# TUMFTM/GraphBasedLocalTrajectoryPlanner

Measured on AMD Instinct MI355X. Metric: planning ticks/s (all action primitives), Monteblanco lattice, higher is better.
Workload: dtype f64; 1 GPU; C2: Monteblanco lattice (128 layers / 2691 nodes / 14264 edges), 4 action primitives, 8 dynamic opponents (16 obstacle positions), sample zone; 32768 independent scenarios per GPU per step, tick pipeline (paths + velocity); batch_per_gpu=32768, batch_total=32768, parallelism=scenario-sharded x1 (no collective; results stay on the ranks)

## Files before the change

graphbasedlocaltrajectoryplanner_amd/csrc/ltpl_hip.hip:

```cpp
#include <hip/hip_runtime.h>
#include <algorithm>
#include <atomic>
#include <cmath>
#include <cstddef>
#include <cstdint>
#include <cstdio>
#include <cstdlib>
#include <cstring>
#include <exception>
#include <memory>
#include <string>
#include <type_traits>
#include <vector>

#include "../../include/ltpl_hip.h"
#include "planner_host.hpp"
#include "fleet_api.hpp"
#include "capsule.hpp"
#include "layer_grid.hpp"
#include "assembly_records.hpp"

#define WG_THREADS 256
#define PIPELINE_MIN_SCEN 64
#define NUM_WAVES 4
// ... 4 lines not shown
#define F_DEF 1
#define F_LEFT 2
#define F_RIGHT 3
#define D_PI 3.14159265358979323846

#define LTPL_SW_PAD 512
struct DevLat {
    int L, V, E, S, G;
    int mode;
    int closed;
    double min_plan_horizon, veh_width, sampled_resolution, lat_offset, vel_decrease_lat, veh_length;
    const int* layer_off; const int* rl_idx;
    const double* s_rl; const double* ref_x; const double* ref_y; const double* vel_rl;
    const double* node_x; const double* node_y; const double* vgoal;
    const int* in_ptr; const int* edge_src; const double* edge_cost; const double* edge_len; const int* samp_ptr;
    const double* sx; const double* sy; const double* spsi; const double* slen;
    const double* ssc;
    const double* glob_rl;
    const double* grx; const double* gry;
    const int* rng_end;
    const int* layer_ebase;
    const unsigned char* edge_src8;
    const unsigned char* edge_dst8;
    const unsigned char* edge_rank8;
    const int* layer_degmax;
    const double* sw_cost;
    const unsigned* sw_meta;
    const int* sw2csc;
    const int* csc2sw;
    const double* b1x; const double* b1y; const double* b2x; const double* b2y; const double* ctx; const double* cty;
    const float4* edge_cap;
    float cull_slack;
    const int4* lgrid; double lg_x0, lg_y0, lg_inv; int lg_nx, lg_ny;
    const int4* node_rec;
    const double* edge_rec;
};

struct DevPathsIn {
    int n_scen, n_w_last;
    const double* w_last;
    const int* start_layer; const int* start_node; const int* flags; const int* last_action; const int* const_closest;
    const double* psi_s;
    const int* veh_off; const int* pos_off; const double* veh_radius; const double* pos_x; const double* pos_y;
    const int* zone_off; const int* zone_gid;
    const int* n_last; const int* last_layer; const int* last_node;
    const int* order;
};

struct DoneSignal { unsigned* host_flag; unsigned* dev_count; unsigned seq; };

__device__ __forceinline__ void signal_done(const DoneSignal& d)
{
    if (!d.host_flag) return;
    __threadfence_system();
    __syncthreads();
    if (threadIdx.x == 0) {
        const unsigned prev = atomicAdd(d.dev_count, 1u);
        if (prev == gridDim.x - 1) {
            *d.dev_count = 0u;
            __hip_atomic_store(d.host_flag, d.seq, __ATOMIC_RELEASE, __HIP_MEMORY_SCOPE_SYSTEM);
        }
    }
}

#ifndef LTPL_VEL_F32_OPERANDS
typedef double ke_scalar;
// ... 555 lines not shown
    const double t = ((px - ax) * (bx - ax) + (py - ay) * (by - ay)) / ((bx - ax) * (bx - ax) + (by - ay) * (by - ay));
    const double fx = ax + t * (bx - ax), fy = ay + t * (by - ay);
    const double ds = sqrt((ax - fx) * (ax - fx) + (ay - fy) * (ay - fy));
    const double s = (ord > 0 ? s_arr[(size_t)i1 * s_stride] : s_arr[(size_t)nb * s_stride]) + ds;
    if (idx0) *idx0 = (ord >= 0) ? i1 : nb;
    return s;
}

__device__ __forceinline__ int globrl_index_dev(const DevLat& lat, double px, double py, int lane)
{
    const int G = lat.G - 1;
    double bd = INFINITY; int nb = 0x7fffffff;
    for (int i0 = 0; i0 < G; i0 += 256) {
        double xs[4], ys[4]; int id[4];
#pragma unroll
        for (int u = 0; u < 4; ++u) { const int i = i0 + u * 64 + lane; id[u] = i < G ? i : G - 1; xs[u] = at(lat.grx, id[u]); ys[u] = at(lat.gry, id[u]); }
#pragma unroll
        for (int u = 0; u < 4; ++u) {
            const double dx = xs[u] - px, dy = ys[u] - py, d2 = dx * dx + dy * dy;
            if (d2 < bd) { bd = d2; nb = id[u]; }
        }
    }
    wave_min2(bd, nb);
    int i1 = nb - 1; if (i1 < 0) i1 += G;
    int i2 = nb + 1; if (i2 > G - 1) i2 = 0;
    const int ord = angle_order_dev(at(lat.grx, nb), at(lat.gry, nb), px, py, at(lat.grx, i1), at(lat.gry, i1), at(lat.grx, i2), at(lat.gry, i2));
    return ord >= 0 ? i1 : nb;
}

__device__ __forceinline__ int lane_globrl_index(const DevLat& lat, double ox, double oy)
{
    const int G = lat.G - 1;
    double bd = INFINITY; int nb = 0;
#pragma unroll 8
    for (int i = 0; i < G; ++i) {
        const double dx = lat.grx[i] - ox, dy = lat.gry[i] - oy, d2 = dx * dx + dy * dy;
        if (d2 < bd) { bd = d2; nb = i; }
    }
    int i1 = nb - 1; if (i1 < 0) i1 += G;
    int i2 = nb + 1; if (i2 > G - 1) i2 = 0;
    const int ord = angle_order_dev(at(lat.grx, nb), at(lat.gry, nb), ox, oy, at(lat.grx, i1), at(lat.gry, i1), at(lat.grx, i2), at(lat.gry, i2));
    return ord >= 0 ? i1 : nb;
}

struct FollowIn { double v_start, v_ego, v_obj, safety_d, obj_dist, obj_x, obj_y; };

template <int EM, bool AXM1, bool GGARR>
__device__ __forceinline__ void follow_profile(const DevLat& lat, int n, int n_el, const VelScratch& vs, double cax, double cay,
                               const DevVelParams& p, const FollowIn& fi, int lane, int* too_close, int* vel_bound,
                               bool ext_sync = false, bool skip_free = false)
{
    int vb = 1;
    const double control_d = p.c_p * fi.safety_d + p.len_veh;
    const double safety_d = fi.safety_d + p.len_veh;
    const int tc = (fi.obj_dist - safety_d) < 0.0;
    const double v_max = p.v_max;

    dbg_stamp(vs.dbg, 4);
    brake_profile<EM, GGARR>(n, vs.wb, vs, cax, cay, fi.v_start, p, lane);
    dbg_stamp(vs.dbg, 5);
    wave_cumsum_seq(vs.el, vs.s, n_el, lane);
    int idb = wave_find_first(n, lane, [&](int i) { return !(vs.wb[i] > 0.01); });
    if (idb > n_el) idb = n_el;
    double ego_stop = 0.0;
    if (idb > 0) ego_stop = (idb < n_el) ? vs.s[idb] : vs.s[n_el - 1] + vs.el[n_el - 1];

    const int G = lat.G - 1;
    const double* grl = lat.glob_rl;
    dbg_stamp(vs.dbg, 6);
    const int idx_s_opp = globrl_index_dev(lat, fi.obj_x, fi.obj_y, lane);
// ... 491 lines not shown
    for (int pass = 0; pass < 4; ++pass) {
        const int half = pass & 1;
        if ((lane >> 5) == half) {
#pragma unroll
            for (int c = 0; c < NCH; c += 2) store2(&E.tbuf[(lane & 31) * PITCH + c], pass < 2 ? vv[c] : aa[c], pass < 2 ? vv[c + 1] : aa[c + 1]);
        }
        wave_sync_lds();
#pragma unroll
        for (int k = 0; k < 4; ++k) {
            const int jl = k * 8 + q, jj = half * 32 + jl, c = 2 * piece;
            const int cn = E.s_cnt[jj];
            if (c >= cn || c >= NCH) continue;
            const dbl2 v = *reinterpret_cast<const dbl2*>(&E.tbuf[jl * PITCH + c]);
            double* o = reinterpret_cast<double*>(E.s_o[jj]) + (pass < 2 ? 0 : E.ax_delta) + (E.s_rhi[jj] - c);
            if (c + 1 < cn) store2_u(o - 1, v.y, v.x); else o[0] = v.x;
        }
        wave_sync_lds();
    }
}

struct NoCap { static constexpr bool active = false; __device__ __forceinline__ double at(int) const { return INFINITY; } };
struct FollowCap {
    static constexpr bool active = true;
    const double* P2; const double* P3; int nd, stop_idx;
    __device__ __forceinline__ double at(int r) const
    {
        const bool from_b = nd < 0 || r < nd - 1;
        const double* src = from_b ? P2 : P3;
        const double v = src[(size_t)r * 64];
        return (!from_b && r > stop_idx) ? 0.0 : v;
    }
};

template <int EM, bool AXM1, bool EMIT = false, class CAP = NoCap>
__device__ __forceinline__ void lane_fb_profile(const LaneProf& L, double* D, int off, int n, double cax, double cay,
                                                const DevVelParams& p, const double* axm_tab, double v_max, double v_start,
                                                bool has_v_end, double v_end, long long* dbg = nullptr, int drow = -1, LaneEmit* em = nullptr, int lane = 0,
                                                const CAP& cap = CAP())
{
    if (v_start < 0.0) v_start = 0.0;
    if (has_v_end && v_end < 0.0) v_end = 0.0;
    const double vmax2 = v_max * v_max, icay = 1.0 / cay, axm1 = axm_tab[1], dm = p.drag_m, axa = fabs(cax);
    const double vend2 = has_v_end ? v_end * v_end : INFINITY;
    const ke_t* KEb = L.KE;
#define KE_AT(r) KEb[kep_row(off + (r))]
    double* Dp = D + (size_t)off * 64;
    const ke_t rec0 = KE_AT(0);
    double kabs_i = (double)rec0.x, e_i = (double)rec0.y;
    double wi = fmin(cay * ke_rcp(rec0), vmax2);
    if (wi > v_start * v_start) wi = v_start * v_start;
    Dp[0] = wi;
    if constexpr (!EMIT) { if (n < 2) return; }
    do {
    if constexpr (EMIT) { if (n < 2) break; }
    if constexpr (EM == 1 && AXM1) {
        constexpr int CA = CAP::active ? LCHC : LCHA;
        const double axg = axa * icay;
        double orig_p = wi, g_p = kabs_i * axg, e_p = e_i;
        bool active = false, prev_acc = false;
        ke_t kr[CA], kn[CA];
        const int nst = n - 1;
#pragma unroll
        for (int c = 0; c < CA; ++c) { const int r = 1 + c < n ? 1 + c : n - 1; kr[c] = KE_AT(r); }
        auto step = [&](const ke_t& rec, int i, bool valid) {
            const double w0n = fmin(cay * ke_rcp(rec), vmax2);
            const bool acc = w0n > orig_p;
            const bool act = active || (acc && !prev_acc);
            const double te = e_p + e_p;
            const double u = fmin(fmax(fma(-g_p, wi, axa), 0.0), axm1);
            const double wn = fmax(fma(te, u, fma(-(te * dm), wi, wi)), 0.0);
            const double wnext = (act && wn < w0n) ? wn : w0n;
            if (valid) {
                Dp[(size_t)(i + 1) * 64] = wnext;
                active = act && !(wn > vmax2); prev_acc = acc;
                wi = wnext; orig_p = w0n; g_p = (double)rec.x * axg; e_p = (double)rec.y;
            }
        };
        int base = 0;
        for (; base + CA <= nst; base += CA) {
#pragma unroll
            for (int c = 0; c < CA; ++c) {
                const int r = base + CA + 1 + c < n ? base + CA + 1 + c : n - 1;
                kn[c] = KE_AT(r);
            }
#pragma unroll
            for (int c = 0; c < CA; ++c) step(kr[c], base + c, true);
// ... 189 lines not shown
                    const double C0 = te * dm, C1 = C0 - te * (axa * kq_n), D1 = te * axa;
                    wn = fmax(fmax(fma(A1, wi, B1), A0 * wi), 0.0);
                    const double t0 = fma(C0, wn, wi), t1 = fma(C1, wn, wi + D1);
                    wn = fmin(fmax(fmax(t1, t0), 0.0), wn);
                } else {
                    const double a = ax_poss_w<EM, AXM1, VMODE_DECEL_BACKW>(wi, kq_i, cax, p, axm_tab, axm1);
                    wn = fmax(wi + 2.0 * a * e_b, 0.0);
                    const double a2 = ax_poss_w<EM, AXM1, VMODE_DECEL_BACKW>(wn, kq_n, cax, p, axm_tab, axm1);
                    wn = fmin(fmax(wi + 2.0 * a2 * e_b, 0.0), wn);
                }
                const bool take = act && wn < wold;
                const double wnext = take ? wn : wold;
                if (valid && take) Dp[(size_t)(n - 2 - i) * 64] = wn;
                const bool act_out = act && !(wn > vmax2);
                active = valid ? act_out : active; prev_acc = valid ? acc : prev_acc;
                orig_i = valid ? wold : orig_i; wi = valid ? wnext : wi; kabs_i = valid ? k_c : kabs_i;
            }
#pragma unroll
            for (int c = 0; c < LCHB; ++c) { kr[c] = kn[c]; wr[c] = wq[c]; }
        }
    }
}

#undef KE_AT

#define VF_BOUND_FOLLOW 1
#define VF_TOO_CLOSE    2
#define VF_HAS_GENERIC  4
#define VF_BOUND_GENERIC 8
#define VF_COMPOSE 16
#define VF_DONE 32

struct LaneFollowOut { int vel_bound, too_close, two_seg, n_decel, stop_idx; };
template <int EM, bool AXM1>
__device__ __forceinline__ LaneFollowOut lane_follow_controlled(const DevLat& lat, const LaneProf& L, double* P2, double* P3, int n, double cax, double cay,
                                                                const DevVelParams& p, const double* axm_tab, double v_start, double v_ego, double v_obj,
                                                                double obj_dist, double safety_d_in, int idx_s_opp, long long* dbg, int drow)
{
    const double icay = 1.0 / cay;
    int vel_bound = 1;
    const double control_d = p.c_p * safety_d_in + p.len_veh, safety_d = safety_d_in + p.len_veh;
    const int too_close = (obj_dist - safety_d) < 0.0 ? 1 : 0;
    const double v_max = p.v_max;
    double v_control;
    if (p.ctrl == 0) v_control = (v_obj - p.k_p * (control_d - obj_dist) + p.k_d * (v_obj - v_ego));
    else {
        double a = (control_d - obj_dist) * D_PI / 2 * 1 / p.tan_w;
        const double lo = -D_PI / 2 + 1e-5, hi = D_PI / 2 - 1e-5;
        a = a < lo ? lo : (a > hi ? hi : a);
        v_control = (v_obj - tan(a) * p.k_p + p.k_d * (v_obj - v_ego));
    }
    if (v_control < 0.0) v_control = 0.0;
    if (v_control > v_max) v_control = v_max;
    const double wctl = v_control * v_control;

    const int G = lat.G - 1;
    const double* grl = lat.glob_rl;
    const double vel0 = grl[(size_t)idx_s_opp * 5 + 4];
    double wopp = fmin(v_obj, vel0); wopp *= wopp;
    double opp_stop = 0.0;
    for (int base = 0; base < G && wopp > 0.01; base += LCH) {
        double kr[LCH], lr[LCH];
#pragma unroll
        for (int c = 0; c < LCH; ++c) {
            int j = base + c + idx_s_opp; j = j % G;
            kr[c] = fabs(grl[(size_t)j * 5 + 3]); lr[c] = grl[(size_t)(j + 1) * 5] - grl[(size_t)j * 5];
        }
#pragma unroll
        for (int c = 0; c < LCH; ++c) {
            const int k = base + c;
            if (k < G && wopp > 0.01) {
                opp_stop += lr[c];
                if (k + 1 >= G) wopp = 0.0;
                else {
                    const double a = ax_poss_w<EM, true, VMODE_DECEL_FORW>(wopp, kr[c] * (1.0 / 14.0), 14.0, p, axm_tab, 0.0);
                    const double r = wopp + 2.0 * a * lr[c];
                    wopp = r < 0.0 ? 0.0 : r;
                }
            }
        }
    }
    vl_stamp(dbg, drow, 1);
    const double s_stop = obj_dist - safety_d + opp_stop;
    double ego_stop = 0.0, s_run = 0.0, s_last = 0.0; int first_le = -1, stop_idx = 0;
    {
        double w = v_start * v_start; bool braking = true, counting = true, searching = true;
        double kr[LCH], er[LCH], kn[LCH], en[LCH];
        auto load_rows = [&](int base, double (&k)[LCH], double (&e)[LCH]) {
#pragma unroll
            for (int c = 0; c < LCH; ++c) {
                const int r = base + c < n ? base + c : n - 1;
                const ke_t ke = L.KE[kep_row(r)]; k[c] = (double)ke.x; e[c] = (double)ke.y;
            }
        };
        load_rows(0, kr, er);
        for (int base = 0; base < n; base += LCH) {
            if (base + LCH < n) load_rows(base + LCH, kn, en);
#pragma unroll
            for (int c = 0; c < LCH; ++c) {
                const int i = base + c;
                if (i < n) {
                    const double wv = braking ? w : 0.0;
                    P2[(size_t)i * 64] = wv;
                    if (first_le < 0 && wv <= wctl) first_le = i;
                    if (counting) { if (wv > 0.01) ego_stop += er[c]; else counting = false; }
                    if (searching) { if (i < n - 1 && s_run < s_stop) stop_idx = i + 1; else searching = false; }
                    if (i == n - 1) s_last = s_run;
                    s_run += er[c];
                    if (braking && i + 1 < n) {
                        const double kq = kr[c] * icay, e = er[c];
                        double r;
                        if constexpr (EM == 1) {
                            const double te = 2.0 * e, axa = fabs(cax);
                            const double A0 = 1.0 - te * p.drag_m, A1 = A0 + te * (axa * kq);
                            r = fmin(fma(A1, w, -te * axa), A0 * w);
                        } else {
                            r = w + 2.0 * ax_poss_w<EM, true, VMODE_DECEL_FORW>(w, kq, cax, p, axm_tab, 0.0) * e;
                        }
// ... 17 lines not shown
                int j = idx + c + idx_s_opp; j = j % G;
                dl[c] = grl[(size_t)(j + 1) * 5] - grl[(size_t)j * 5];
            }
#pragma unroll
            for (int c = 0; c < LCH; ++c)
                if (run) { if (summed < s_ends && idx < G) { summed += dl[c]; ++idx; } else run = false; }
            if (run && !(summed < s_ends && idx < G)) run = false;
        }
        int j = (idx % G) + idx_s_opp; if (j >= G) j -= G;
        v_end = grl[(size_t)j * 5 + 4];
    }
    vl_stamp(dbg, drow, 3);
    int idx_c = 0, n_decel = 0; const bool two_seg = ego_stop < s_stop;
    if (two_seg) {
        double vcs = v_start;
        if (v_start > v_control && stop_idx >= 2) {
            idx_c = first_le < 0 ? 0 : first_le;
            if (idx_c > stop_idx) idx_c = stop_idx;
            if (idx_c == 0) idx_c = stop_idx;
            n_decel = idx_c + 1 < n ? idx_c + 1 : n;
            vcs = sqrt(P2[(size_t)(n_decel - 1) * 64]);
        } else if (!(stop_idx >= 2)) vel_bound = 0;
        const int m = (stop_idx + 1 < n ? stop_idx + 1 : n) - idx_c;
        if (stop_idx - idx_c > 0) {
            lane_fb_profile<EM, AXM1>(L, P3, idx_c, m, cax, cay, p, axm_tab, v_control, vcs, true, v_end);
            if (fabs(sqrt(P3[(size_t)idx_c * 64]) - vcs) > 1.0) vel_bound = 0;
        } else if (stop_idx - idx_c == 0) P3[(size_t)idx_c * 64] = vcs * vcs;
        const double first_v = (n_decel - 1 > 0) ? sqrt(P2[0]) : sqrt(P3[0]);
        if (fabs(first_v - v_start) > 1.0) vel_bound = 0;
    }
    vl_stamp(dbg, drow, 4);
    LaneFollowOut o; o.vel_bound = vel_bound; o.too_close = too_close; o.two_seg = two_seg ? 1 : 0; o.n_decel = n_decel; o.stop_idx = stop_idx;
    return o;
}

template <int EM, bool AXM1>
__device__ __forceinline__ int lane_generic_profile(const DevLat& lat, const DevPathsOut& out, const LaneProf& L, double* D, int slot, int n,
                                    int reduced, double cax, double cay, const DevVelParams& p, const double* axm_tab,
                                    double vel_plan, double v_max_offset)
{
    const int goal = out.goal_layer[slot];
    const int end_node = out.nodes[(size_t)slot * out.cap_nodes + out.n_nodes[slot] - 1];
    int dn = end_node - lat.rl_idx[goal]; if (dn < 0) dn = -dn;
    const double raceline_offset = (double)dn * lat.lat_offset;
    double v_end; int v_idx;
    if (reduced) {
        v_end = 0.0;
        double spl_len = 0.0;
        for (int i = 0; i < n - 1; ++i) spl_len += (double)L.KE[kep_row(i)].y;
        int first = -1; double c = 0.0;
        for (int i = 0; i < n - 1; ++i) { c += (double)L.KE[kep_row(i)].y; if (first < 0 && !(c < (spl_len - 5.0))) first = i; }
        v_idx = (first < 0 ? 0 : first) + 1;
        if (v_idx == 1 && n > 1) v_idx = n;
    } else {
        v_end = lat.vel_rl[goal];
        const double red = v_end * lat.vel_decrease_lat * raceline_offset;
        v_end -= (red < v_end ? red : v_end);
        v_idx = n;
    }
    if (v_idx > 1) lane_fb_profile<EM, AXM1>(L, D, 0, v_idx, cax, cay, p, axm_tab, p.v_max, vel_plan, true, v_end);
    else D[0] = 0.0;
    for (int i = (v_idx > 1 ? v_idx : 1); i < n; ++i) D[(size_t)i * 64] = 0.0;
    return fabs(sqrt(D[0]) - vel_plan) < v_max_offset ? 1 : 0;
}

template <int EM, bool AXM1>
// ... 85 lines not shown
        LaneProf L; L.KE = vp.KE + kep_base(j, vp.plane_rows);
        double* o_vx = vout.vx + (size_t)slot * out.cap_pts;
        le_o[lane] = have ? (unsigned long long)o_vx : 0ull;
        LaneEmit E; E.tbuf = le_tbuf; E.s_cnt = le_cnt; E.s_rhi = le_rhi; E.s_o = le_o; E.ax_delta = (long long)(vout.ax - vout.vx); E.w0 = 0.0;
        wave_sync_lds();
        const int bound = lane_generic_profile_emit<EM, AXM1>(lat, out, L, vp.P0 + tile_base(j, vp.cap_pts), have, slot, n, have ? out.reduced[slot] : 0,
                                                              cax, cay, p, axm_tab, have ? vin.vel_plan[slot / LTPL_MAX_ACTIONS] : 0.0, vin.v_max_offset, E, lane, o_vx);
        if (have) {
            vout.vel_bound[slot] = bound; vout.too_close[slot] = 0;
            vp.flags[j] = VF_BOUND_FOLLOW | (bound ? VF_BOUND_GENERIC : 0);
        }
        vl_stamp(dbg, drow, 6);
        return;
    }
    if (b >= nbG && (emit & 2)) {
        const int j = (b - nbG) * 64 + lane;
        const bool have = j < cntF;
        const int tile = fbase + j;
        const int2 js = have ? out.job_slot[tile] : make_int2(0, 0);
        const int slot = js.x, n = have ? js.y : 0;
        {
            const int nmax = wave_max_i32(n);
            if (lane == 0) atomicMax(&out.job_cnt[2], nmax);
        }
        const int s = slot / LTPL_MAX_ACTIONS;
        LaneProf L; L.KE = vp.KE + kep_base(tile, vp.plane_rows);
        double* P2 = vp.P2 + tile_base(j, vp.cap_pts);
        double* P3 = vp.P3 + tile_base(j, vp.cap_pts);
        const double vel_plan = have ? vin.vel_plan[s] : 0.0;
        const int reduced = have ? out.reduced[slot] : 0;
        FollowCap cap; cap.P2 = P2; cap.P3 = P3; cap.nd = -1; cap.stop_idx = 0;
        bool direct = false;
        int o_bound = 0, o_close = 0;
        if (have) {
            const LaneFollowOut fo = lane_follow_controlled<EM, AXM1>(lat, L, P2, P3, n, cax, cay, p, axm_tab, vel_plan, vin.vel_est[s], prep.v_obj[slot],
                                                                      prep.obj_dist[slot], vin.safety_d, prep.idx_s_opp[slot], dbg, drow);
            o_bound = fo.vel_bound; o_close = fo.too_close;
            if (!reduced) { direct = true; cap.nd = fo.two_seg ? fo.n_decel : -1; cap.stop_idx = fo.stop_idx; }
            else {
                double* P0 = vp.P0 + tile_base(tile, vp.cap_pts);
                int flags = VF_BOUND_FOLLOW | VF_HAS_GENERIC;
                if (fo.too_close) flags |= VF_TOO_CLOSE;
                if (!fo.vel_bound) flags &= ~VF_BOUND_FOLLOW;
                const bool two_seg = fo.two_seg != 0;
                for (int i = 0; i < n; ++i) {
                    const bool from_b = !two_seg || i < fo.n_decel - 1;
                    P0[(size_t)i * 64] = from_b ? P2[(size_t)i * 64] : ((i > fo.stop_idx) ? 0.0 : P3[(size_t)i * 64]);
                }
                if (lane_generic_profile<EM, AXM1>(lat, out, L, P3, slot, n, reduced, cax, cay, p, axm_tab, vel_plan, vin.v_max_offset))
                    flags |= VF_BOUND_GENERIC;
                vp.flags[tile] = flags;
            }
        }
        double* o_vx = vout.vx + (size_t)slot * out.cap_pts;
        le_o[lane] = direct ? (unsigned long long)o_vx : 0ull;
        LaneEmit E; E.tbuf = le_tbuf; E.s_cnt = le_cnt; E.s_rhi = le_rhi; E.s_o = le_o; E.ax_delta = (long long)(vout.ax - vout.vx); E.w0 = 0.0;
        wave_sync_lds();
        double* D = direct ? vp.P1 + tile_base(j, vp.cap_pts) : P2;
        lane_fb_profile<EM, AXM1, true, FollowCap>(L, D, 0, direct && n >= 2 ? n : 0, cax, cay, p, axm_tab, p.v_max, vel_plan, false, 0.0, nullptr, -1, &E, lane, cap);
        if (direct) {
            const int i = n - 1;
            const double w = fmin(cap.at(i), D[(size_t)i * 64]);
            o_vx[i] = sqrt(w); o_vx[i + E.ax_delta] = 0.0;
            vout.vel_bound[slot] = o_bound; vout.too_close[slot] = o_close;
            vp.flags[tile] = VF_DONE;
        }
        vl_stamp(dbg, drow, 6);
        return;
    }
    const bool fjob = b >= nbG;
    const int j = (fjob ? b - nbG : b) * 64 + lane;
    if (j >= (fjob ? cntF : cntG)) return;
    const int tile = fjob ? fbase + j : j;
    const int2 js = out.job_slot[tile];
    const int slot = js.x;
    {
        int nmax = js.y;
#pragma unroll
        for (int m = 32; m >= 1; m >>= 1) { const int o = __shfl_xor(nmax, m); nmax = o > nmax ? o : nmax; }
        if (lane == 0) atomicMax(&out.job_cnt[2], nmax);
    }
    const int s = slot / LTPL_MAX_ACTIONS;
    const int n = js.y;
    LaneProf L; L.KE = vp.KE + kep_base(tile, vp.plane_rows);
    double* P0 = vp.P0 + tile_base(tile, vp.cap_pts);
    double* P2 = vp.P2 + tile_base(fjob ? j : 0, vp.cap_pts);
    double* P3 = vp.P3 + tile_base(fjob ? j : 0, vp.cap_pts);
    const double vel_plan = vin.vel_plan[s];
    const int name = out.action_id[slot], reduced = out.reduced[slot];
    int flags = VF_BOUND_FOLLOW;

    if (name == LTPL_ACT_FOLLOW) {
// ... 690 lines not shown

    ltpl_handle* h = new ltpl_handle();
    h->device = device;
    h->rng_end_host = rng_end;
    struct Guard { ltpl_handle* h; ~Guard() { if (h) ltpl_destroy(h); } } guard{h};
    auto fail = [&](int code) { g_create_error = h->err; return code; };
    if (hipSetDevice(device) != hipSuccess) { h->err = "hipSetDevice failed"; return fail(LTPL_ERR_HIP); }
    if (hipStreamCreateWithFlags(&h->stream, hipStreamNonBlocking) != hipSuccess) { h->err = "hipStreamCreate failed"; return fail(LTPL_ERR_HIP); }

    DevLat& L = h->lat;
    L.L = d->num_layers; L.V = d->num_nodes; L.E = d->num_edges; L.S = d->num_samples; L.G = d->num_glob_rl;
    L.mode = d->plan_horizon_mode; L.closed = d->closed ? 1 : 0; L.min_plan_horizon = d->min_plan_horizon; L.veh_width = d->veh_width;
    L.sampled_resolution = d->sampled_resolution; L.lat_offset = d->lat_offset;
    L.vel_decrease_lat = d->vel_decrease_lat; L.veh_length = d->veh_length;
#define UP(field, src, n) if ((rc = upload(h, src, (size_t)(n), &L.field)) != LTPL_OK) return fail(rc)
    UP(layer_off, d->layer_node_off, L.L + 1); UP(rl_idx, d->raceline_index, L.L);
    UP(s_rl, d->s_raceline, L.L); UP(ref_x, d->refline_x, L.L); UP(ref_y, d->refline_y, L.L);
    UP(vel_rl, d->vel_raceline, L.L);
    UP(node_x, d->node_x, L.V); UP(node_y, d->node_y, L.V); UP(vgoal, d->vgoal_cost, L.V);
    UP(in_ptr, d->in_ptr, L.V + 1); UP(edge_src, d->edge_src, L.E);
    UP(edge_cost, d->edge_cost, L.E);
    UP(edge_len, d->edge_len, L.E); UP(samp_ptr, d->samp_ptr, L.E + 1);
    UP(sx, d->samp_x, L.S); UP(sy, d->samp_y, L.S); UP(spsi, d->samp_psi, L.S); UP(slen, d->samp_len, L.S);
    UP(glob_rl, d->glob_rl, (size_t)L.G * 5);
    {
        std::vector<double> sc(2 * (size_t)L.S + 2, 0.0);
        for (int k = 0; k < L.S; ++k) { sc[2 * (size_t)k] = sin(d->samp_psi[k]); sc[2 * (size_t)k + 1] = cos(d->samp_psi[k]); }
        UP(ssc, sc.data(), 2 * (size_t)L.S + 2);
    }
    {
        std::vector<double> gx((size_t)L.G), gy((size_t)L.G);
        for (int k = 0; k < L.G; ++k) { gx[(size_t)k] = d->glob_rl[(size_t)k * 5 + 1]; gy[(size_t)k] = d->glob_rl[(size_t)k * 5 + 2]; }
        UP(grx, gx.data(), L.G); UP(gry, gy.data(), L.G);
    }
    {
        std::vector<int> ebase((size_t)L.L + 1);
        for (int l = 0; l <= L.L; ++l) ebase[(size_t)l] = d->in_ptr[d->layer_node_off[l]];
        std::vector<unsigned char> src8((size_t)L.E + 16, (unsigned char)0xff);
        for (int e = 0; e < L.E; ++e) src8[(size_t)e] = (unsigned char)d->edge_src[e];
        std::vector<unsigned char> dst8((size_t)L.E);
        for (int l = 0; l < L.L; ++l)
            for (int v = d->layer_node_off[l]; v < d->layer_node_off[l + 1]; ++v)
                for (int e = d->in_ptr[v]; e < d->in_ptr[v + 1]; ++e) dst8[(size_t)e] = (unsigned char)(v - d->layer_node_off[l]);
        UP(rng_end, rng_end.data(), L.L); UP(layer_ebase, ebase.data(), L.L + 1); UP(edge_src8, src8.data(), L.E + 16);
        UP(edge_dst8, dst8.data(), L.E);
        std::vector<unsigned char> rank8((size_t)L.E);
        for (int v = 0; v < L.V; ++v)
            for (int e = d->in_ptr[v]; e < d->in_ptr[v + 1]; ++e) rank8[(size_t)e] = (unsigned char)(e - d->in_ptr[v]);
        UP(edge_rank8, rank8.data(), L.E);
        {
            std::vector<int32_t> nrec; std::vector<double> erec;
            ltplrec::build(L.V, L.E, d->in_ptr, d->edge_src, d->edge_len, d->samp_ptr, d->samp_x, d->samp_y, d->samp_psi, nrec, erec);
            const int4* nr = nullptr;
            if ((rc = upload(h, reinterpret_cast<const int4*>(nrec.data()), (size_t)L.V, &nr)) != LTPL_OK) return fail(rc);
            L.node_rec = nr;
            UP(edge_rec, erec.data(), (size_t)L.E * LTPL_EDGE_REC);
        }
        std::vector<int> ldeg((size_t)L.L, 0);
        for (int l = 0; l < L.L; ++l)
            for (int v = d->layer_node_off[l]; v < d->layer_node_off[l + 1]; ++v)
                ldeg[(size_t)l] = std::max(ldeg[(size_t)l], d->in_ptr[v + 1] - d->in_ptr[v]);
        UP(layer_degmax, ldeg.data(), L.L);
        h->sw2csc_host.resize((size_t)L.E);
        std::vector<int> csc2sw((size_t)L.E);
        for (int l = 0; l < L.L; ++l) {
            const int e0 = ebase[(size_t)l], e1 = ebase[(size_t)l + 1];
// ... 690 lines not shown
    if (polled) done = next_done_signal(h);
    hipLaunchKernelGGL(kern, dim3(n_jobs), dim3(64), lds, h->stream, h->lat, p,
                       reinterpret_cast<const DevVelJob*>(db + o_jobs), reinterpret_cast<const double*>(db + o_pool),
                       reinterpret_cast<double*>(dob + o_vx), reinterpret_cast<int*>(dob + o_flags), cap, h->lp4.dbg, done, 1);
    HIP_TRY(h, hipGetLastError());
    if (!zc) HIP_TRY(h, hipMemcpyAsync(h->h_out, h->d_out, aout.size, hipMemcpyDeviceToHost, h->stream));
    prof_enq.stop();
    LTPL_PROF(prof_sync, "vel_profile.sync");
    if (polled) { if ((rc = wait_done(h, done.seq))) return rc; }
    else HIP_TRY(h, hipStreamSynchronize(h->stream));
    prof_sync.stop();
    dbg_report(h, "k_vel_profile", n_jobs);
    LTPL_PROF(prof_sc, "vel_profile.scatter");
    const unsigned char* ho = static_cast<const unsigned char*>(h->h_out);
    const int* flags = reinterpret_cast<const int*>(ho + o_flags);
    const double* vx = reinterpret_cast<const double*>(ho + o_vx);
    for (int j = 0; j < n_jobs; ++j) {
        memcpy(results[j].vx, vx + dj[(size_t)j].off_out, sizeof(double) * (size_t)jobs[j].n);
        results[j].too_close = flags[2 * j]; results[j].vel_bound = flags[2 * j + 1];
    }
    return LTPL_OK;
} LTPL_ABI_CATCH(abi_err_of(h))

struct TickLayout {
    InLayout in; size_t axm, vel_plan, vel_est, pos_x, pos_y, veh_vel, in_total;
    OutLayout out; size_t vx, ax, vel_bound, too_close, out_total;
    int n_scen, cap_nodes, cap_pts;
    DevPathsIn di; DevPathsOut dout; DevVelParams p; DevTickVelIn dvin; DevTickVelOut dvout;
    int vel_off, vel_stride, vel_cap; size_t lds;
    int variant;
    bool pipeline; size_t prep_odist, prep_vobj, prep_ox, prep_oy, prep_idx; size_t planes_bytes;
    DevVelPrep dprep; int prep_off, prep_stride;
    VelPlanes vp{}; int n_slots_pad = 0, n_scen_pad = 0;
};

static int tick_prepare(ltpl_handle* h, const ltpl_paths_in* in, const ltpl_tick_vel_in* vin, int cap_nodes, int cap_pts,
                        TickLayout* t)
{
    int rc = validate_and_layout(h, in, &t->in);
    if (rc) return rc;
    if (!vin || !vin->params) { h->err = "velocity inputs missing"; return LTPL_ERR_INVALID_ARG; }
    if (cap_nodes < h->caps.max_path_nodes || cap_pts < h->caps.max_path_pts) { h->err = "output capacity too small"; return LTPL_ERR_CAPACITY; }
    const int n = in->n_scen;
    for (int s = 0; s < n; ++s)
        if (vin->vel_plan[s] > vin->params->v_max + 0.1) {
            h->err = "vel_plan > v_max + 0.1: the brake-prefix branch is not part of the fused tick (the reference raises at OTH.py:919)";
            return LTPL_ERR_UNSUPPORTED;
        }
    t->n_scen = n; t->cap_nodes = cap_nodes; t->cap_pts = cap_pts;
    t->variant = vel_variant(vin->params);
    Arena a; a.size = t->in.total;
    t->axm = a.add(sizeof(double) * 2 * (size_t)vin->params->n_ax_max_machines);
    t->vel_plan = a.add(sizeof(double) * (size_t)n); t->vel_est = a.add(sizeof(double) * (size_t)n);
    t->pos_x = a.add(sizeof(double) * (size_t)n); t->pos_y = a.add(sizeof(double) * (size_t)n);
    t->veh_vel = a.add(sizeof(double) * (size_t)(t->in.n_veh + 1));
    t->in_total = a.size;
    layout_out(n, cap_nodes, cap_pts, &t->out);
    Arena b; b.size = t->out.total;
    t->vx = b.add(sizeof(double) * (size_t)n * LTPL_MAX_ACTIONS * (size_t)cap_pts);
    t->ax = b.add(sizeof(double) * (size_t)n * LTPL_MAX_ACTIONS * (size_t)cap_pts);
    t->vel_bound = b.add(sizeof(int) * (size_t)n * LTPL_MAX_ACTIONS);
    t->too_close = b.add(sizeof(int) * (size_t)n * LTPL_MAX_ACTIONS);
    t->pipeline = h->long_horizon || (!h->force_fused && (!h->fused_fits || n >= h->pipeline_min_scen));
    t->prep_odist = b.add(sizeof(double) * (size_t)n * LTPL_MAX_ACTIONS);
    t->prep_vobj = b.add(sizeof(double) * (size_t)n * LTPL_MAX_ACTIONS);
    t->prep_ox = b.add(sizeof(double) * (size_t)n * LTPL_MAX_ACTIONS);
// ... 45 lines not shown

static int tick_pack(ltpl_handle* h, const ltpl_paths_in* in, const ltpl_tick_vel_in* vin, TickLayout* t,
                     unsigned char* hb, unsigned char* db, unsigned char* dob)
{
    pack_in(in, t->in, hb, db, &t->di, h->scen_order != 0);
    const int n = in->n_scen;
    memcpy(hb + t->axm, vin->params->ax_max_machines, sizeof(double) * 2 * (size_t)vin->params->n_ax_max_machines);
    memcpy(hb + t->vel_plan, vin->vel_plan, sizeof(double) * (size_t)n);
    memcpy(hb + t->vel_est, vin->vel_est, sizeof(double) * (size_t)n);
    memcpy(hb + t->pos_x, vin->pos_est_x, sizeof(double) * (size_t)n);
    memcpy(hb + t->pos_y, vin->pos_est_y, sizeof(double) * (size_t)n);
    if (t->in.n_veh > 0) memcpy(hb + t->veh_vel, vin->veh_vel, sizeof(double) * (size_t)t->in.n_veh);
    int rc = make_vel_params(h, vin->params, reinterpret_cast<const double*>(db + t->axm), &t->p);
    if (rc) return rc;
    t->dvin.gg_ax = vin->gg_ax; t->dvin.gg_ay = vin->gg_ay; t->dvin.safety_d = vin->safety_d;
    t->dvin.v_max_offset = vin->v_max_offset;
    t->dvin.vel_plan = reinterpret_cast<const double*>(db + t->vel_plan);
    t->dvin.vel_est = reinterpret_cast<const double*>(db + t->vel_est);
    t->dvin.pos_est_x = reinterpret_cast<const double*>(db + t->pos_x);
    t->dvin.pos_est_y = reinterpret_cast<const double*>(db + t->pos_y);
    t->dvin.veh_vel = reinterpret_cast<const double*>(db + t->veh_vel);
    if (t->pipeline && t->planes_bytes > h->d_planes_cap) {
        if (h->d_planes) (void)hipFree(h->d_planes);
        h->d_planes = nullptr; h->d_planes_cap = 0;
        HIP_TRY(h, hipMalloc(&h->d_planes, t->planes_bytes));
        h->d_planes_cap = t->planes_bytes;
    }
    tick_bind_outputs(t, dob, static_cast<double*>(h->d_planes));
    return LTPL_OK;
}

static int tick_launch_paths(ltpl_handle* h, const TickLayout& t, hipStream_t st)
{
    if (t.dout.job_cnt) HIP_TRY(h, hipMemsetAsync(t.dout.job_cnt, 0, 3 * sizeof(int), st));
    return launch_paths(h, (t.n_scen >= h->nw1_min_scen && h->batch_nw == 1) ? 1 : NUM_WAVES, t.n_scen, st, t.di, t.dout);
}

static int tick_launch_vel(ltpl_handle* h, const TickLayout& t, hipStream_t st, hipEvent_t ev_after_prep = nullptr)
{
    HIP_TRY(h, hipMemsetAsync(t.dvout.vel_bound, 0, sizeof(int) * (size_t)t.n_scen * LTPL_MAX_ACTIONS, st));
    HIP_TRY(h, hipMemsetAsync(t.dvout.too_close, 0, sizeof(int) * (size_t)t.n_scen * LTPL_MAX_ACTIONS, st));
#ifdef LTPL_EXPERIMENT
    if (!(h->exp_skip & 1))
#endif
    hipLaunchKernelGGL(k_follow_prep, dim3((t.n_scen + 63) / 64), dim3(64), 0, st, h->lat, t.di, t.dout,
                       t.dvin, t.dprep, t.vp, t.n_scen, h->lp4.dbg);
    HIP_TRY(h, hipGetLastError());
    if (ev_after_prep) HIP_TRY(h, hipEventRecord(ev_after_prep, st));
    const int n_slots = t.n_scen * LTPL_MAX_ACTIONS;
    const int nb0 = (n_slots + 63) / 64, nb1 = (t.n_scen + 63) / 64;
    const int emit_generic = t.n_scen >= LTPL_EMIT_MIN_SCEN ? 1 : 0;
    const int emit = emit_generic | ((emit_generic && t.n_scen >= h->follow_emit_min_scen) ? 2 : 0);
#ifdef LTPL_EXPERIMENT
    if (!(h->exp_skip & 2))
#endif
    hipLaunchKernelGGL(lanes_kernel_of(t.variant), dim3(nb0 + 2 * nb1), dim3(64), 0, st, h->lat, t.di, t.dout,
                       t.p, t.dvin, t.dprep, t.vp, n_slots, t.n_scen, nb0, h->lp4.dbg, t.dvout, emit);
    HIP_TRY(h, hipGetLastError());
#ifdef LTPL_EXPERIMENT
    if (!(h->exp_skip & 4))
#endif
    hipLaunchKernelGGL(k_vel_final, dim3(emit_generic ? nb1 : nb0 + nb1, h->final_y), dim3(64), 0, st, t.dout, t.dvin, t.dvout, t.vp, n_slots, t.n_scen,
                       emit_generic ? nb0 : 0);
    HIP_TRY(h, hipGetLastError());
    return LTPL_OK;
}

static int tick_launch(ltpl_handle* h, const TickLayout& t, hipEvent_t* ev = nullptr)
// ... 355 lines not shown
    if (!h) return LTPL_ERR_INVALID_ARG;
    if (!h->resident) { h->err = "no resident batch: call ltpl_batch_upload first"; return LTPL_ERR_INVALID_ARG; }
    if (reps < 1) { h->err = "reps < 1"; return LTPL_ERR_INVALID_ARG; }
    HIP_TRY(h, hipSetDevice(h->device));
    hipEvent_t e0 = nullptr, e1 = nullptr;
    if (ms_total) {
        HIP_TRY(h, hipEventCreate(&e0)); HIP_TRY(h, hipEventCreate(&e1));
        HIP_TRY(h, hipEventRecord(e0, h->stream));
    }
    if (h->resident_x[0] && ms_total) {
        while (h->ev_step.size() < 2 * (size_t)reps) { hipEvent_t e; HIP_TRY(h, hipEventCreate(&e)); h->ev_step.push_back(e); }
    }
    h->last_paths_ms = 0.0f; h->last_paths_n = 0;
    if (h->resident_x[0]) {
        constexpr int K = ltpl_handle::PIPE_SETS;
        const bool two = h->path_streams == 2 && h->path_stream2;
        if (two) {
            HIP_TRY(h, hipEventRecord(h->ev_begin, h->stream));
            HIP_TRY(h, hipStreamWaitEvent(h->path_stream2, h->ev_begin, 0));
        }
        for (int r = 0; r < reps; ++r) {
            const int set = r % K;
            const TickLayout& T = set ? *h->resident_x[set - 1] : *h->resident;
            hipStream_t sp = (two && (r & 1)) ? h->path_stream2 : h->stream;
            if (r >= K) HIP_TRY(h, hipStreamWaitEvent(sp, h->ev_vel[set], 0));
            if (ms_total) HIP_TRY(h, hipEventRecord(h->ev_step[2 * (size_t)r], sp));
            int rc = tick_launch_paths(h, T, sp);
            if (rc) return rc;
            if (ms_total) HIP_TRY(h, hipEventRecord(h->ev_step[2 * (size_t)r + 1], sp));
            HIP_TRY(h, hipEventRecord(h->ev_paths[set], sp));
            hipStream_t sv = h->vel_stream[r % ltpl_handle::VEL_STREAMS];
            HIP_TRY(h, hipStreamWaitEvent(sv, h->ev_paths[set], 0));
            if ((rc = tick_launch_vel(h, T, sv))) return rc;
            HIP_TRY(h, hipEventRecord(h->ev_vel[set], sv));
            h->last_set = set;
        }
        for (int i = 0; i < K && i < reps; ++i) HIP_TRY(h, hipStreamWaitEvent(h->stream, h->ev_vel[i], 0));
    } else {
        for (int r = 0; r < reps; ++r) { int rc = tick_launch(h, *h->resident); if (rc) return rc; }
    }
    if (ms_total) {
        HIP_TRY(h, hipEventRecord(e1, h->stream));
        HIP_TRY(h, hipEventSynchronize(e1));
        HIP_TRY(h, hipEventElapsedTime(ms_total, e0, e1));
        (void)hipEventDestroy(e0); (void)hipEventDestroy(e1);
        if (h->resident_x[0]) {
            for (int r = 0; r < reps; ++r) {
                float ms = 0.0f;
                HIP_TRY(h, hipEventElapsedTime(&ms, h->ev_step[2 * (size_t)r], h->ev_step[2 * (size_t)r + 1]));
                h->last_paths_ms += ms;
            }
            h->last_paths_n = reps;
        }
    } else {
        HIP_TRY(h, hipStreamSynchronize(h->stream));
    }
    return LTPL_OK;
} LTPL_ABI_CATCH(abi_err_of(h))

extern "C" int ltpl_batch_last_paths_ms(ltpl_handle* h, float* ms_avg)
{
    if (!h || !ms_avg) return LTPL_ERR_INVALID_ARG;
    *ms_avg = h->last_paths_n > 0 ? h->last_paths_ms / (float)h->last_paths_n : 0.0f;
    return LTPL_OK;
}

// ... 389 lines not shown
```

Measured before the change: 40.48 million ticks/s.

## Add raceline grid lookup, fuse follow forward sweep, move counter clears to vel stream

Three separate changes. A spatial grid over the global raceline replaces the brute-force nearest-point scan over all G points per lane with a scan of candidate cells. The follow-controlled braking walk now also computes the forward acceleration sweep into P1 in the same pass, so the later profile call skips its forward loop and starts from the precomputed sweep. The job-counter memset moves from the paths stream to the end of the vel stream, taking it off the paths critical path. Risks: the grid candidate sets must cover the true nearest point, and the fused sweep must match the old forward-pass semantics.

New measurement: 37.49 million ticks/s. 0.926x the previous value.

```diff
diff --git a/graphbasedlocaltrajectoryplanner_amd/csrc/ltpl_hip.hip b/graphbasedlocaltrajectoryplanner_amd/csrc/ltpl_hip.hip
--- a/graphbasedlocaltrajectoryplanner_amd/csrc/ltpl_hip.hip
+++ b/graphbasedlocaltrajectoryplanner_amd/csrc/ltpl_hip.hip
@@ -60,6 +60,7 @@
     const float4* edge_cap;
     float cull_slack;
     const int4* lgrid; double lg_x0, lg_y0, lg_inv; int lg_nx, lg_ny;
+    const int4* rgrid; double rg_x0, rg_y0, rg_inv; int rg_nx, rg_ny;
     const int4* node_rec;
     const double* edge_rec;
 };
@@ -681,10 +682,33 @@
 {
     const int G = lat.G - 1;
     double bd = INFINITY; int nb = 0;
+    int4 c = make_int4(0, -1, 0, 0);
+    if (lat.rgrid != nullptr) {
+        const double fx = (ox - lat.rg_x0) * lat.rg_inv, fy = (oy - lat.rg_y0) * lat.rg_inv;
+        if (fx >= 0.0 && fy >= 0.0 && fx < (double)lat.rg_nx && fy < (double)lat.rg_ny) c = lat.rgrid[(int)fy * lat.rg_nx + (int)fx];
+    }
+    if (c.y >= 0) {
+        const int tot = c.y + c.w;
+        for (int k0 = 0; k0 < tot; k0 += 4) {
+            int l4[4]; double x4[4], y4[4];
+#pragma unroll
+            for (int u = 0; u < 4; ++u) {
+                const int k = k0 + u < tot ? k0 + u : tot - 1;
+                l4[u] = k < c.y ? c.x + k : c.z + (k - c.y);
+                x4[u] = at(lat.grx, l4[u]); y4[u] = at(lat.gry, l4[u]);
+            }
+#pragma unroll
+            for (int u = 0; u < 4; ++u) {
+                const double dx = x4[u] - ox, dy = y4[u] - oy, d2 = dx * dx + dy * dy;
+                if (d2 < bd) { bd = d2; nb = l4[u]; }
+            }
+        }
+    } else {
 #pragma unroll 8
-    for (int i = 0; i < G; ++i) {
-        const double dx = lat.grx[i] - ox, dy = lat.gry[i] - oy, d2 = dx * dx + dy * dy;
-        if (d2 < bd) { bd = d2; nb = i; }
+        for (int i = 0; i < G; ++i) {
+            const double dx = lat.grx[i] - ox, dy = lat.gry[i] - oy, d2 = dx * dx + dy * dy;
+            if (d2 < bd) { bd = d2; nb = i; }
+        }
     }
     int i1 = nb - 1; if (i1 < 0) i1 += G;
     int i2 = nb + 1; if (i2 > G - 1) i2 = 0;
@@ -1242,12 +1266,13 @@
     }
 };
 
-template <int EM, bool AXM1, bool EMIT = false, class CAP = NoCap>
+template <int EM, bool AXM1, bool EMIT = false, class CAP = NoCap, bool PREFWD = false>
 __device__ __forceinline__ void lane_fb_profile(const LaneProf& L, double* D, int off, int n, double cax, double cay,
                                                 const DevVelParams& p, const double* axm_tab, double v_max, double v_start,
                                                 bool has_v_end, double v_end, long long* dbg = nullptr, int drow = -1, LaneEmit* em = nullptr, int lane = 0,
                                                 const CAP& cap = CAP())
 {
+    static_assert(!PREFWD || EMIT, "the forward sweep is only handed in to the form with direct output");
     if (v_start < 0.0) v_start = 0.0;
     if (has_v_end && v_end < 0.0) v_end = 0.0;
     const double vmax2 = v_max * v_max, icay = 1.0 / cay, axm1 = axm_tab[1], dm = p.drag_m, axa = fabs(cax);
@@ -1255,13 +1280,21 @@
     const ke_t* KEb = L.KE;
 #define KE_AT(r) KEb[kep_row(off + (r))]
     double* Dp = D + (size_t)off * 64;
-    const ke_t rec0 = KE_AT(0);
-    double kabs_i = (double)rec0.x, e_i = (double)rec0.y;
-    double wi = fmin(cay * ke_rcp(rec0), vmax2);
-    if (wi > v_start * v_start) wi = v_start * v_start;
-    Dp[0] = wi;
+    double kabs_i, wi;
+    [[maybe_unused]] double e_i = 0.0;
+    if constexpr (PREFWD) {
+        const int r = n >= 1 ? n - 1 : 0;
+        kabs_i = (double)KE_AT(r).x; wi = Dp[(size_t)r * 64];
+    } else {
+        const ke_t rec0 = KE_AT(0);
+        kabs_i = (double)rec0.x; e_i = (double)rec0.y;
+        wi = fmin(cay * ke_rcp(rec0), vmax2);
+        if (wi > v_start * v_start) wi = v_start * v_start;
+        Dp[0] = wi;
+    }
     if constexpr (!EMIT) { if (n < 2) return; }
     do {
+    if constexpr (PREFWD) break;
     if constexpr (EMIT) { if (n < 2) break; }
     if constexpr (EM == 1 && AXM1) {
         constexpr int CA = CAP::active ? LCHC : LCHA;
@@ -1517,10 +1550,97 @@
 #define VF_DONE 32
 
 struct LaneFollowOut { int vel_bound, too_close, two_seg, n_decel, stop_idx; };
+
 template <int EM, bool AXM1>
+__device__ __forceinline__ void lane_follow_forward_walk(const LaneProf& L, double* P2, double* P1, bool fwd, int n, double cax, double cay, const DevVelParams& p,
+                                                         const double* axm_tab, double v_start, double wctl, double s_stop,
+                                                         double& ego_stop, double& s_last, int& first_le, int& stop_idx)
+{
+    const double icay = 1.0 / cay, axa = fabs(cax), dm = p.drag_m;
+    const double vs_f = v_start < 0.0 ? 0.0 : v_start;
+    const double vmax2 = p.v_max * p.v_max, axm1 = axm_tab[1], axg = axa * icay;
+    const ke_t rec0 = L.KE[kep_row(0)];
+    double kabs_i = (double)rec0.x, e_i = (double)rec0.y;
+    double wi = fmin(cay * ke_rcp(rec0), vmax2);
+    if (wi > vs_f * vs_f) wi = vs_f * vs_f;
+    if (fwd) P1[0] = wi;
+    double orig_p = wi, g_p = kabs_i * axg;
+    bool active = false, prev_acc = false;
+    double w = v_start * v_start, s_run = 0.0; bool braking = true, counting = true, searching = true;
+    ke_t kr[LCH], kn[LCH];
+    auto load_rows = [&](int base, ke_t (&k)[LCH]) {
+#pragma unroll
+        for (int c = 0; c < LCH; ++c) { const int r = base + c < n ? base + c : n - 1; k[c] = L.KE[kep_row(r)]; }
+    };
+    load_rows(0, kr);
+    for (int base = 0; base < n; base += LCH) {
+        load_rows(base + LCH, kn);
+#pragma unroll
+        for (int c = 0; c < LCH; ++c) {
+            const int i = base + c;
+            const bool valid = i < n;
+            const ke_t rec = kr[c];
+            const double k_c = (double)rec.x, e_c = (double)rec.y;
+            {
+                const bool fv = fwd && valid && i >= 1;
+                double w0n, wn; bool acc;
+                if constexpr (EM == 1 && AXM1) {
+                    w0n = fmin(cay * ke_rcp(rec), vmax2);
+                    acc = w0n > orig_p;
+                    const double te = e_i + e_i;
+                    const double u = fmin(fmax(fma(-g_p, wi, axa), 0.0), axm1);
+                    wn = fmax(fma(te, u, fma(-(te * dm), wi, wi)), 0.0);
+                } else {
+                    w0n = fast_div(cay, k_c);
+                    w0n = (w0n < vmax2) ? w0n : vmax2;
+                    acc = w0n - orig_p > 0.0;
+                    const double kq_i = kabs_i * icay;
+                    const double a = ax_poss_w<EM, AXM1, VMODE_ACCEL_FORW>(wi, kq_i, cax, p, axm_tab, axm1);
+                    wn = fmax(wi + 2.0 * a * e_i, 0.0);
+                }
+                const bool act = active || (acc && !prev_acc);
+                const double wnext = (act && wn < w0n) ? wn : w0n;
+                if (fv) P1[(size_t)i * 64] = wnext;
+                active = fv ? (act && !(wn > vmax2)) : active; prev_acc = fv ? acc : prev_acc;
+                wi = fv ? wnext : wi; orig_p = fv ? w0n : orig_p;
+                g_p = fv ? k_c * axg : g_p; kabs_i = fv ? k_c : kabs_i; e_i = fv ? e_c : e_i;
+            }
+            {
+                const double wv = braking ? w : 0.0;
+                if (valid) P2[(size_t)i * 64] = wv;
+                first_le = (valid && first_le < 0 && wv <= wctl) ? i : first_le;
+                const bool cnt = counting && wv > 0.01;
+                ego_stop = (valid && cnt) ? ego_stop + e_c : ego_stop;
+                counting = valid ? cnt : counting;
+                const bool adv = searching && i < n - 1 && s_run < s_stop;
+                stop_idx = (valid && adv) ? i + 1 : stop_idx;
+                searching = valid ? adv : searching;
+                s_last = (valid && i == n - 1) ? s_run : s_last;
+                s_run = valid ? s_run + e_c : s_run;
+                const double kq = k_c * icay;
+                double r;
+                if constexpr (EM == 1) {
+                    const double te = 2.0 * e_c;
+                    const double A0 = 1.0 - te * p.drag_m, A1 = A0 + te * (axa * kq);
+                    r = fmin(fma(A1, w, -te * axa), A0 * w);
+                } else {
+                    r = w + 2.0 * ax_poss_w<EM, true, VMODE_DECEL_FORW>(w, kq, cax, p, axm_tab, 0.0) * e_c;
+                }
+                const bool st = valid && braking && i + 1 < n;
+                braking = (st && r < 0.0) ? false : braking;
+                w = (st && !(r < 0.0)) ? r : w;
+            }
+        }
+#pragma unroll
+        for (int c = 0; c < LCH; ++c) kr[c] = kn[c];
+    }
+}
+
+template <int EM, bool AXM1, bool FUSE_FWD = false>
 __device__ __forceinline__ LaneFollowOut lane_follow_controlled(const DevLat& lat, const LaneProf& L, double* P2, double* P3, int n, double cax, double cay,
                                                                 const DevVelParams& p, const double* axm_tab, double v_start, double v_ego, double v_obj,
-                                                                double obj_dist, double safety_d_in, int idx_s_opp, long long* dbg, int drow)
+                                                                double obj_dist, double safety_d_in, int idx_s_opp, long long* dbg, int drow,
+                                                                double* P1 = nullptr, bool fwd_on = false)
 {
     const double icay = 1.0 / cay;
     int vel_bound = 1;
@@ -1568,7 +1688,9 @@
     vl_stamp(dbg, drow, 1);
     const double s_stop = obj_dist - safety_d + opp_stop;
     double ego_stop = 0.0, s_run = 0.0, s_last = 0.0; int first_le = -1, stop_idx = 0;
-    {
+    if constexpr (FUSE_FWD) {
+        lane_follow_forward_walk<EM, AXM1>(L, P2, P1, fwd_on, n, cax, cay, p, axm_tab, v_start, wctl, s_stop, ego_stop, s_last, first_le, stop_idx);
+    } else {
         double w = v_start * v_start; bool braking = true, counting = true, searching = true;
         double kr[LCH], er[LCH], kn[LCH], en[LCH];
         auto load_rows = [&](int base, double (&k)[LCH], double (&e)[LCH]) {
@@ -1652,6 +1774,15 @@
     vl_stamp(dbg, drow, 4);
     LaneFollowOut o; o.vel_bound = vel_bound; o.too_close = too_close; o.two_seg = two_seg ? 1 : 0; o.n_decel = n_decel; o.stop_idx = stop_idx;
     return o;
+}
+
+template <int EM, bool AXM1>
+__device__ __forceinline__ LaneFollowOut lane_follow_fused(const DevLat& lat, const LaneProf& L, double* P2, double* P3, double* P1, bool fwd_on, int n,
+                                                           double cax, double cay, const DevVelParams& p, const double* axm_tab, double v_start, double v_ego,
+                                                           double v_obj, double obj_dist, double safety_d_in, int idx_s_opp, long long* dbg, int drow)
+{
+    return lane_follow_controlled<EM, AXM1, true>(lat, L, P2, P3, n, cax, cay, p, axm_tab, v_start, v_ego, v_obj, obj_dist, safety_d_in, idx_s_opp, dbg, drow,
+                                                  P1, fwd_on);
 }
 
 template <int EM, bool AXM1>
@@ -1803,9 +1934,10 @@
         FollowCap cap; cap.P2 = P2; cap.P3 = P3; cap.nd = -1; cap.stop_idx = 0;
         bool direct = false;
         int o_bound = 0, o_close = 0;
+        double* P1 = vp.P1 + tile_base(j, vp.cap_pts);
         if (have) {
-            const LaneFollowOut fo = lane_follow_controlled<EM, AXM1>(lat, L, P2, P3, n, cax, cay, p, axm_tab, vel_plan, vin.vel_est[s], prep.v_obj[slot],
-                                                                      prep.obj_dist[slot], vin.safety_d, prep.idx_s_opp[slot], dbg, drow);
+            const LaneFollowOut fo = lane_follow_fused<EM, AXM1>(lat, L, P2, P3, P1, !reduced, n, cax, cay, p, axm_tab, vel_plan, vin.vel_est[s], prep.v_obj[slot],
+                                                                 prep.obj_dist[slot], vin.safety_d, prep.idx_s_opp[slot], dbg, drow);
             o_bound = fo.vel_bound; o_close = fo.too_close;
             if (!reduced) { direct = true; cap.nd = fo.two_seg ? fo.n_decel : -1; cap.stop_idx = fo.stop_idx; }
             else {
@@ -1827,8 +1959,8 @@
         le_o[lane] = direct ? (unsigned long long)o_vx : 0ull;
         LaneEmit E; E.tbuf = le_tbuf; E.s_cnt = le_cnt; E.s_rhi = le_rhi; E.s_o = le_o; E.ax_delta = (long long)(vout.ax - vout.vx); E.w0 = 0.0;
         wave_sync_lds();
-        double* D = direct ? vp.P1 + tile_base(j, vp.cap_pts) : P2;
-        lane_fb_profile<EM, AXM1, true, FollowCap>(L, D, 0, direct && n >= 2 ? n : 0, cax, cay, p, axm_tab, p.v_max, vel_plan, false, 0.0, nullptr, -1, &E, lane, cap);
+        double* D = P1;
+        lane_fb_profile<EM, AXM1, true, FollowCap, true>(L, D, 0, direct && n >= 2 ? n : 0, cax, cay, p, axm_tab, p.v_max, vel_plan, false, 0.0, nullptr, -1, &E, lane, cap);
         if (direct) {
             const int i = n - 1;
             const double w = fmin(cap.at(i), D[(size_t)i * 64]);
@@ -2585,6 +2717,14 @@
         std::vector<double> gx((size_t)L.G), gy((size_t)L.G);
         for (int k = 0; k < L.G; ++k) { gx[(size_t)k] = d->glob_rl[(size_t)k * 5 + 1]; gy[(size_t)k] = d->glob_rl[(size_t)k * 5 + 2]; }
         UP(grx, gx.data(), L.G); UP(gry, gy.data(), L.G);
+        L.rgrid = nullptr; L.rg_x0 = L.rg_y0 = L.rg_inv = 0.0; L.rg_nx = L.rg_ny = 0;
+        if (L.G - 1 >= 1 && !getenv("LTPL_NO_RACELINE_GRID")) {
+            const ltplgrid::Grid g = ltplgrid::build(L.G - 1, gx.data(), gy.data());
+            if (g.nx > 0 && g.ny > 0) {
+                UP(rgrid, reinterpret_cast<const int4*>(g.cells.data()), (size_t)g.nx * g.ny);
+                L.rg_x0 = g.x0; L.rg_y0 = g.y0; L.rg_inv = g.inv_cell; L.rg_nx = g.nx; L.rg_ny = g.ny;
+            }
+        }
     }
     {
         std::vector<int> ebase((size_t)L.L + 1);
@@ -3341,6 +3481,7 @@
     bool pipeline; size_t prep_odist, prep_vobj, prep_ox, prep_oy, prep_idx; size_t planes_bytes;
     DevVelPrep dprep; int prep_off, prep_stride;
     VelPlanes vp{}; int n_slots_pad = 0, n_scen_pad = 0;
+    mutable bool counters_clear = false;
 };
 
 static int tick_prepare(ltpl_handle* h, const ltpl_paths_in* in, const ltpl_tick_vel_in* vin, int cap_nodes, int cap_pts,
@@ -3452,8 +3593,17 @@
 
 static int tick_launch_paths(ltpl_handle* h, const TickLayout& t, hipStream_t st)
 {
-    if (t.dout.job_cnt) HIP_TRY(h, hipMemsetAsync(t.dout.job_cnt, 0, 3 * sizeof(int), st));
+    if (t.dout.job_cnt && !t.counters_clear) HIP_TRY(h, hipMemsetAsync(t.dout.job_cnt, 0, 3 * sizeof(int), st));
+    t.counters_clear = false;
     return launch_paths(h, (t.n_scen >= h->nw1_min_scen && h->batch_nw == 1) ? 1 : NUM_WAVES, t.n_scen, st, t.di, t.dout);
+}
+
+static int tick_clear_counters(ltpl_handle* h, const TickLayout& t, hipStream_t st)
+{
+    if (!t.dout.job_cnt) return LTPL_OK;
+    HIP_TRY(h, hipMemsetAsync(t.dout.job_cnt, 0, 3 * sizeof(int), st));
+    t.counters_clear = true;
+    return LTPL_OK;
 }
 
 static int tick_launch_vel(ltpl_handle* h, const TickLayout& t, hipStream_t st, hipEvent_t ev_after_prep = nullptr)
@@ -3875,6 +4025,7 @@
             hipStream_t sv = h->vel_stream[r % ltpl_handle::VEL_STREAMS];
             HIP_TRY(h, hipStreamWaitEvent(sv, h->ev_paths[set], 0));
             if ((rc = tick_launch_vel(h, T, sv))) return rc;
+            if ((rc = tick_clear_counters(h, T, sv))) return rc;
             HIP_TRY(h, hipEventRecord(h->ev_vel[set], sv));
             h->last_set = set;
         }
```
